# AMReX-Combustion/PeleAnalysis

Measured on AMD Instinct MI355X. Metric: Mcells/s for grad+curvature on 512^3-base 3-level AMR; % HBM roofline, higher is better.
Workload: dtype f64; 1 GPU; fused grad->curvature, 3-level AMR, base 512^3, ref_ratio 2, 128^3 boxes (64 per level) in the file, swept on the internal tiling pa_level_retile makes of them (4, 4, 4 boxes per level, largest 512x256x256), 1 comp(s), periodic x/y + wall z, 402653184 cells in the job; cells=402653184, cells_this_rank=402653184, ncomp=1, components_per_batch=1, fused=True, parallelism=single GPU

## Files before the change

### peleanalysis_amd/csrc/pa_core.hip

```cpp
#include "pa_internal.h"
#include "pa_dist.h"
#include <algorithm>
#include <atomic>
#include <cstring>
#include <numeric>

int pa_fail(pa_ctx* ctx, const std::string& msg) {
  if (ctx) ctx->err = msg;
  return 1;
}

int pa_ensure_scr(pa_ctx* ctx, size_t bytes, int slot) {
  void*& p = slot ? ctx->d_scr2 : ctx->d_scr;
  size_t& cap = slot ? ctx->scr2_cap : ctx->scr_cap;
  if (cap >= bytes) return 0;
  if (p) (void)hipFree(p);
  p = nullptr;
  cap = 0;
  PA_HIP(hipMalloc(&p, bytes));
  cap = bytes;
  return 0;
}

extern "C" int pa_version(void) { return 100; }

static int host_owner(const pa_level* L, int i, int j, int k);
const WgTab* pa_sweep_wgtab(const pa_level* L, int cls, int tw, int mty, int kseg, bool force, int part) {
  if (part) force = true;
  const long long key = ((long long)cls << 56) | ((long long)part << 54) | ((long long)(force ? 1 : 0) << 52) | ((long long)tw << 40) | ((long long)mty << 24) | (long long)kseg;
  auto it = L->wgtabs.find(key);
  if (it != L->wgtabs.end()) return (it->second->d || part) ? it->second.get() : nullptr;
  std::unique_ptr<WgTab> T(new WgTab());
  struct Chunk { int n, box, t0; };
  std::vector<std::pair<int, int>> bt;
  std::vector<std::vector<int>> sel;
  long long real = 0;
  int tmax = 0;
  std::vector<unsigned char> sp;
  if (part) {
    sp.assign(L->boxes.size(), 0);
    for (int f : L->sfaces) sp[(size_t)(f / 6)] |= (unsigned char)(1u << (f % 6));
  }
  for (int b = 0; b < (int)L->boxes.size(); ++b) {
    const DBox& B = L->boxes[b];
    const int nx = B.hi[0] - B.lo[0] + 1, ny = B.hi[1] - B.lo[1] + 1, nz = B.hi[2] - B.lo[2] + 1;
    if (cls != 2 && (nx <= 32) != (cls == 1)) continue;
    const int tx = (nx + tw - 1) / tw, ty = (ny + mty - 1) / mty, tz = (nz + kseg - 1) / kseg;
    int t = tx * ty * tz;
    if (part) {
      std::vector<int> mine;
      for (int id = 0; id < t; ++id) {
        const int bx = id % tx, by = (id / tx) % ty, bz = id / (tx * ty);
        int lo[3] = {B.lo[0] + bx * tw, B.lo[1] + by * mty, B.lo[2] + bz * kseg}, hi[3];
        hi[0] = std::min(lo[0] + tw - 1, B.hi[0]); hi[1] = std::min(lo[1] + mty - 1, B.hi[1]); hi[2] = std::min(lo[2] + kseg - 1, B.hi[2]);
        bool early = true;
        for (int d = 0; d < 3 && early; ++d) {
          if (((sp[(size_t)b] >> (2 * d)) & 1) && lo[d] == B.lo[d]) early = false;
          if (((sp[(size_t)b] >> (2 * d + 1)) & 1) && hi[d] >= B.hi[d] - 1) early = false;
        }
        for (int d = 0; d < 3 && early; ++d)
          for (int side = 0; side < 2 && early; ++side) {
            int slo[3], shi[3];
            for (int q = 0; q < 3; ++q) { slo[q] = std::max(lo[q] - 2, B.lo[q] - 2); shi[q] = std::min(hi[q] + 2, B.hi[q] + 2); }
            if (side == 0) shi[d] = std::min(shi[d], B.lo[d] - 1); else slo[d] = std::max(slo[d], B.hi[d] + 1);
            if (slo[d] > shi[d]) continue;
            for (int k = slo[2]; k <= shi[2] && early; ++k)
              for (int j = slo[1]; j <= shi[1] && early; ++j)
                for (int i = slo[0]; i <= shi[0]; ++i)
                  if (host_owner(L, i, j, k) < 0) { early = false; break; }
          }
        if (early == (part == 1)) mine.push_back(id);
      }
      t = (int)mine.size();
      if (t == 0) continue;
      sel.push_back(std::move(mine));
    }
    bt.push_back({t, b});
    real += t;
    tmax = std::max(tmax, t);
  }
  const long long launched = (long long)tmax * 8 * (((long long)bt.size() + 7) / 8);
  if (!bt.empty()) {
    constexpr int chunk_env = 0;
    const int cap = chunk_env > 0 ? chunk_env : (int)std::max<long long>(8, std::min<long long>(64, real / 32));
    std::vector<Chunk> ch;
    for (size_t bi = 0; bi < bt.size(); ++bi) {
      const auto& p = bt[bi];
      const int parts = (p.first + cap - 1) / cap;
      for (int q = 0; q < parts; ++q) {
        const int a = (int)((long long)p.first * q / parts), e = (int)((long long)p.first * (q + 1) / parts);
        ch.push_back({e - a, part ? (int)bi : p.second, a});
      }
    }
    std::stable_sort(ch.begin(), ch.end(), [](const Chunk& a, const Chunk& b) { return a.n > b.n; });
    std::vector<Chunk> queue[8];
    long long load[8] = {0, 0, 0, 0, 0, 0, 0, 0};
    for (const Chunk& c : ch) {
      int q = 0;
      for (int x = 1; x < 8; ++x)
        if (load[x] < load[q]) q = x;
      queue[q].push_back(c);
      load[q] += c.n;
    }
    const long long qlen = *std::max_element(load, load + 8);
    if (force || launched * 100 > qlen * 8 * 103) {
      std::vector<int> tab((size_t)(qlen * 8 * 2), 0);
      for (int q = 0; q < 8; ++q) {
        long long s = 0;
        for (const Chunk& c : queue[q])
          for (int t = 0; t < c.n; ++t, ++s) {
            tab[(size_t)(2 * (8 * s + q))] = part ? bt[(size_t)c.box].second : c.box;
            tab[(size_t)(2 * (8 * s + q) + 1)] = part ? sel[(size_t)c.box][(size_t)(c.t0 + t)] : c.t0 + t;
          }
        for (; s < qlen; ++s) tab[(size_t)(2 * (8 * s + q))] = -1;
      }
      if (hipMalloc(&T->d, sizeof(int) * tab.size()) == hipSuccess && hipMemcpy(T->d, tab.data(), sizeof(int) * tab.size(), hipMemcpyHostToDevice) == hipSuccess) {
        T->n = (unsigned)(tab.size() / 2);
        T->h = std::move(tab);
      } else {
        if (T->d) (void)hipFree(T->d);
        T->d = nullptr;
        (void)hipGetLastError();
      }
    }
  }
  const WgTab* raw = T.get();
  L->wgtabs[key] = std::move(T);
  return (raw->d || part) ? raw : nullptr;
}

const unsigned char* pa_sweep_gneed(const pa_level* L, const WgTab* T, int tw, int mty, int kseg, long long fine_serial, const std::vector<int>* cpregs) {
  if (!T || !T->d || T->h.size() != 2 * (size_t)T->n) return nullptr;
  auto it = T->gneed.find(fine_serial);
  if (it != T->gneed.end()) return it->second;
  const int nb = (int)L->boxes.size();
  pa_level* Lm = const_cast<pa_level*>(L);
  if ((int)Lm->xneed.size() != nb) {
    std::vector<unsigned char> sp((size_t)nb, 0);
    for (int f : L->sfaces) sp[(size_t)(f / 6)] |= (unsigned char)(1u << (f % 6));
    Lm->xneed.assign((size_t)nb, 0);
    for (int b = 0; b < nb; ++b) {
      const DBox& B = L->boxes[b];
      for (int side = 0; side < 2; ++side) {
        bool need = (sp[(size_t)b] >> side) & 1;
        const int x = side ? B.hi[0] + 1 : B.lo[0] - 1;
        int last = -1;
        for (int k = B.lo[2]; k <= B.hi[2] && !need; k += L->g)
          for (int j = B.lo[1]; j <= B.hi[1] && !need; j += L->g) {
            const int o = host_owner(L, x, j, k);
            if (o < 0 || o == last) continue;
            last = o;
            const DBox& N = L->boxes[o];
            if ((sp[(size_t)o] >> (1 - side)) & 1) need = true;
            for (int d = 1; d < 3 && !need; ++d)
              for (int t = 0; t < 2; ++t) {
                const int c = t ? N.hi[d] : N.lo[d];
                if (((sp[(size_t)o] >> (2 * d + t)) & 1) && c >= B.lo[d] + 3 && c <= B.hi[d] - 3) need = true;
              }
          }
        if (need) Lm->xneed[(size_t)b] |= (unsigned char)(2u << side);
      }
    }
  }
  std::vector<std::vector<unsigned char>> full((size_t)nb);
  auto tiles = [&](const DBox& B, int& tx, int& ty, int& tz) {
    tx = (B.hi[0] - B.lo[0] + tw) / tw; ty = (B.hi[1] - B.lo[1] + mty) / mty; tz = (B.hi[2] - B.lo[2] + kseg) / kseg;
  };
  if (cpregs)
    for (size_t r = 0; r + 12 <= cpregs->size(); r += 12) {
      const int* R = cpregs->data() + r;
      const int sb = R[1], dir = R[9], t0 = dir == 0 ? 1 : 0, t1 = dir == 2 ? 1 : 2;
      if (sb < 0 || sb >= nb) continue;
      const DBox& B = L->boxes[sb];
      int lo[3] = {R[4], R[5], R[6]}, hi[3] = {R[4], R[5], R[6]};
      hi[t0] += R[7] - 1; hi[t1] += R[8] - 1;
      int tx, ty, tz;
      tiles(B, tx, ty, tz);
      auto& F = full[(size_t)sb];
      if (F.empty()) F.assign((size_t)tx * ty * tz, 0);
      const int a0 = std::max(0, (lo[0] - B.lo[0]) / tw), a1 = std::min(tx - 1, (hi[0] - B.lo[0]) / tw);
      const int b0 = std::max(0, (lo[1] - B.lo[1]) / mty), b1 = std::min(ty - 1, (hi[1] - B.lo[1]) / mty);
      const int c0 = std::max(0, (lo[2] - B.lo[2]) / kseg), c1 = std::min(tz - 1, (hi[2] - B.lo[2]) / kseg);
      for (int c = c0; c <= c1; ++c)
        for (int bb = b0; bb <= b1; ++bb)
          for (int a = a0; a <= a1; ++a) F[((size_t)c * ty + bb) * tx + a] = 1;
    }
  std::vector<unsigned char> need((size_t)T->n, 0);
  for (unsigned e = 0; e < T->n; ++e) {
    const int b = T->h[2 * (size_t)e], id = T->h[2 * (size_t)e + 1];
    if (b < 0 || b >= nb) continue;
    unsigned char v = Lm->xneed[(size_t)b];
    if (!full[(size_t)b].empty() && id >= 0 && (size_t)id < full[(size_t)b].size() && full[(size_t)b][(size_t)id]) v |= 1;
    need[(size_t)e] = v;
  }
  unsigned char* d = nullptr;
  if (hipMalloc(&d, need.size()) != hipSuccess || hipMemcpy(d, need.data(), need.size(), hipMemcpyHostToDevice) != hipSuccess) {
    if (d) (void)hipFree(d);
    (void)hipGetLastError();
    return nullptr;
  }
  T->gneed[fine_serial] = d;
  return d;
}

static pa_options g_opt;
static bool g_opt_read = false;
extern "C" void pa_options_reload(void) {
  pa_options o;
  auto geti = [](const char* n, int def) { const char* e = getenv(n); return e ? atoi(e) : def; };
  o.filter_exact = geti("PA_FILTER_EXACT", 0) != 0;
  o.allow_unverified_gaussian = geti("PA_ALLOW_UNVERIFIED_GAUSSIAN", 0) != 0;
  if (const char* e = getenv("PA_RETILE_MAX")) {
    int v[3] = {0, 0, 0};
    if (sscanf(e, "%d %d %d", &v[0], &v[1], &v[2]) == 3 && v[0] > 0 && v[1] > 0 && v[2] > 0)
      for (int d = 0; d < 3; ++d) o.retile_max[d] = v[d];
  }
  o.fused2 = geti("PA_FUSED2", 1) != 0;
  o.ncg = geti("PA_NCG", 1) != 0;
  o.dist_early = geti("PA_DIST_EARLY", 0) != 0;
  o.smooth_replicated = geti("PA_SMOOTH_REPLICATED", 0) != 0;
  o.smooth_mg = geti("PA_SMOOTH_MG", -1);
  o.smooth_march = geti("PA_SMOOTH_MARCH", 1) != 0;
  o.smooth_timing = geti("PA_SMOOTH_TIMING", 0) != 0;
  o.force_fallbacks = geti("PA_FORCE_FALLBACKS", 0) != 0;
  o.scratch_poison = geti("PA_SCRATCH_POISON", 0) != 0;
  g_opt = o;
  g_opt_read = true;
}
const pa_options& pa_opt() {
  if (!g_opt_read) pa_options_reload();
  return g_opt;
}

extern "C" pa_ctx* pa_ctx_create(int device, void* hip_stream) {
  int ndev = 0;
  if (hipGetDeviceCount(&ndev) != hipSuccess || ndev <= 0 || device >= ndev) return nullptr;
  if (hipSetDevice(device) != hipSuccess) return nullptr;
  pa_ctx* ctx = new pa_ctx();
  ctx->device = device;
  if (hip_stream) {
    ctx->stream = (hipStream_t)hip_stream;
  } else {
    if (hipStreamCreate(&ctx->stream) != hipSuccess) { delete ctx; return nullptr; }
    ctx->own_stream = true;
  }
  if (hipMalloc(&ctx->d_flags, 16 * sizeof(int)) != hipSuccess || hipMemset(ctx->d_flags, 0, 16 * sizeof(int)) != hipSuccess) {
    if (ctx->own_stream) (void)hipStreamDestroy(ctx->stream);
    delete ctx;
    return nullptr;
  }
  if (hipStreamCreateWithFlags(&ctx->stream2, hipStreamNonBlocking) != hipSuccess) { ctx->stream2 = nullptr; (void)hipGetLastError(); }
  return ctx;
}

extern "C" void pa_ctx_destroy(pa_ctx* ctx) {
  PaBind bind_(ctx);
  if (!ctx) return;
  pa_rccl_destroy(ctx);
  if (ctx->d_red) (void)hipFree(ctx->d_red);
  if (ctx->d_flags) (void)hipFree(ctx->d_flags);
  if (ctx->d_slow) (void)hipFree(ctx->d_slow);
  if (ctx->d_prog) (void)hipFree(ctx->d_prog);
  for (hipEvent_t e : ctx->fix_evs)
    if (e) (void)hipEventDestroy(e);
  if (ctx->d_scr) (void)hipFree(ctx->d_scr);
  if (ctx->d_scr2) (void)hipFree(ctx->d_scr2);
  if (ctx->h_pin) (void)hipHostFree(ctx->h_pin);
  if (ctx->d_mcz) (void)hipFree(ctx->d_mcz);
  if (ctx->d_flat_nosrc) (void)hipFree(ctx->d_flat_nosrc);
  for (auto& c : ctx->surf_cache) (void)hipFree(c.first);
  for (auto& e : ctx->evs) { (void)hipEventDestroy(e.a); (void)hipEventDestroy(e.b); }
  for (auto& e : ctx->sync_evs) (void)hipEventDestroy(e);
  if (ctx->stream2) (void)hipStreamDestroy(ctx->stream2);
  for (auto& st : ctx->lev_streams) (void)hipStreamDestroy(st);
  if (ctx->own_stream) (void)hipStreamDestroy(ctx->stream);
  delete ctx;
}

extern "C" int pa_profile_enable(pa_ctx* ctx, int on) {
  PaBind bind_(ctx);
  if (!ctx) return 1;
// ... 1103 lines not shown
```

### peleanalysis_amd/csrc/pa_internal.h

```cpp
#pragma once
#include <hip/hip_runtime.h>
#include <cstdint>
#include <array>
#include <map>
#include <memory>
#include <string>
#include <utility>
#include <vector>
#include "../../include/peleanalysis_amd.h"

struct DBox { int lo[3]; int hi[3]; };

struct pa_options {
  int filter_exact = 0;
  int allow_unverified_gaussian = 0;
  int retile_max[3] = {0, 0, 0};
  int fused2 = 1;
  int ncg = 1;
  int dist_early = 0;
  int smooth_replicated = 0;
  int smooth_mg = -1;
  int smooth_march = 1;
  int smooth_timing = 0;
  int scratch_poison = 0;
// ... 37 lines not shown

struct DMFView {
  double* data;
  const long long* off;
  int ncomp, ng;
  int xform;
  double xa, xb;
};

#define PA_MAXB 4
#define PA_MAXSLOTS 16
template <typename A, int CAP = PA_MAXB>
struct LevBatch {
  int n = 0;
  int ycum[CAP + 1] = {};
  A a[CAP];
  __device__ __forceinline__ int find(unsigned y, unsigned& local) const {
    int l = 0;
    while (l + 1 < n && y >= (unsigned)ycum[l + 1]) ++l;
    local = y - (unsigned)ycum[l];
    return l;
  }
};

struct pa_ctx {
  int device = 0;
  hipStream_t stream = nullptr;
  bool own_stream = false;
  std::string err;
  double* d_red = nullptr;
  size_t red_cap = 0;
  int* d_flags = nullptr;
  void* d_slow = nullptr;
  hipEvent_t fix_evs[2] = {nullptr, nullptr};
  double* d_prog = nullptr;
  void* d_scr = nullptr;
  size_t scr_cap = 0;
  void* d_scr2 = nullptr;
  size_t scr2_cap = 0;
  void* h_pin = nullptr;
  size_t h_pin_cap = 0;
  void* d_mcz = nullptr;
  size_t mcz_cap = 0;
  bool mcz_dirty = true;
  std::map<void*, size_t> surf_live;
  std::vector<std::pair<void*, size_t>> surf_cache;
  unsigned profile = 0;
  struct Ev { hipEvent_t a, b; int tag; };
  std::vector<Ev> evs;
  hipStream_t stream2 = nullptr;
  std::vector<hipStream_t> lev_streams;
  std::vector<hipEvent_t> sync_evs;
  std::string sweep_kernel;
  int smooth_iters = -1;
  double smooth_res = 0.0;
  int curv_path = -1;
  unsigned long long* d_flat_nosrc = nullptr;
  int32_t filter_info[8] = {0, 0, 0, 0, 0, 0, 0, 0};
  pa_comm comm = {nullptr, 0, 1, nullptr, nullptr};
  struct RcclState* rccl = nullptr;
};

struct ProfScope {
  pa_ctx* ctx;
  pa_ctx::Ev e;
  bool on;
  ProfScope(pa_ctx* c, int tag) : ctx(c), on(((c->profile >> tag) & 1u) != 0) {
    if (!on) return;
    e.tag = tag;
    if (hipEventCreate(&e.a) != hipSuccess || hipEventCreate(&e.b) != hipSuccess) { on = false; return; }
    (void)hipEventRecord(e.a, ctx->stream);
  }
  ~ProfScope() {
    if (!on) return;
    (void)hipEventRecord(e.b, ctx->stream);
    ctx->evs.push_back(e);
  }
};
enum { PA_TAG_GRADCURV = 1, PA_TAG_GRADCURV_FACES = 2, PA_TAG_FILL = 3, PA_TAG_BC = 4, PA_TAG_GRAD = 5, PA_TAG_PROGRESS = 6,
       PA_TAG_FILTER = 7, PA_TAG_MC = 8, PA_TAG_XCHG = 9 };

struct WgTab {
  int* d = nullptr;
  unsigned n = 0;
  std::vector<int> h;
  mutable std::map<long long, unsigned char*> gneed;
  ~WgTab() {
    if (d) (void)hipFree(d);
    for (auto& kv : gneed)
      if (kv.second) (void)hipFree(kv.second);
  }
};

struct pa_level {
  pa_ctx* ctx = nullptr;
  std::vector<DBox> boxes;
  int domlo[3], domhi[3], is_per[3];
  double prob_lo[3], prob_hi[3], dx[3], dxinv[3];
  int g = 1, mlo[3], mn[3];
  std::vector<int> owner;
  DBox* d_boxes = nullptr;
  int* d_owner = nullptr;
  std::vector<int> sfaces;
  int* d_sfaces = nullptr;
  int* d_sfindex = nullptr;
  long long* d_sfoff = nullptr;
  unsigned short* d_sfcode = nullptr;
  int maxn[3] = {0, 0, 0};
  long long ncells = 0;
  bool fusable = true;
  bool pure_faces = true;
  long long* d_cpoff = nullptr;
  double* d_cp = nullptr;
  int cp_sets = 0, cg_sets = 0;
  long long cp_total = 0;
  long long* d_cgoff = nullptr;
  double* d_cg = nullptr;
  long long cg_total = 0;
  double* d_ncg = nullptr;
  bool ncg_live = false;
  int ncg_minw = 0;
  std::vector<long long> cgoff;
  int* d_blist = nullptr;
  int nwide = 0, nnarrow = 0;
  int wmax[3] = {0, 0, 0}, nmax[3] = {0, 0, 0};
  int* d_sfboxes = nullptr;
  int nsfboxes = 0;
  void* d_sfwg = nullptr;
  int nsfwg = 0;
  void* d_pfwg = nullptr;
  int npfwg = 0;
  SfChunk* d_sfchunk = nullptr;
  int nsfchunk = 0;
  void* d_ring = nullptr;
  int nring = -1;
  std::vector<unsigned char> xneed;
  void* d_irr = nullptr;
  int nirr = -1;
  int nremote = 0;
  DLevelView view;
  int rank = 0, nranks = 1;
  long long serial = 0;
  std::vector<DBox> gboxes;
  std::vector<int> gowner;
  std::vector<int> gid;
  std::vector<int> glocal;
  bool source_only = false;
  mutable std::map<int, std::unique_ptr<struct XPlan>> fb_plans;
  mutable std::map<long long, std::unique_ptr<struct CpPlan>> cp_plans;
  mutable std::map<int, std::unique_ptr<struct FbLocal>> fb_local;
  mutable std::map<std::pair<long long, int>, std::unique_ptr<struct CsPlan>> cs_plans;
  mutable std::unique_ptr<struct RepPlan> rep_plan;
  mutable std::map<long long, std::unique_ptr<WgTab>> wgtabs;
  mutable std::map<long long, std::unique_ptr<struct RsPlan>> rs_plans;
  mutable std::map<std::pair<long long, int>, std::unique_ptr<struct FpPlan>> fp_plans;
  mutable std::map<std::array<long long, 5>, std::unique_ptr<struct FlPlan>> fl_plans;
  mutable std::map<std::array<int, 3>, struct pa_mf*> scratch;
  ~pa_level();
};

struct FpPlan {
  int n = 0;
  void* d_items = nullptr;
  ~FpPlan();
};

struct FlPlan {
  int nwide = 0, ngeneral = 0, nskipped = 0, nrect = 0;
  int nptile = 0, notile = 0, ngtile = 0;
  void* d_ptile = nullptr;
  void* d_rects = nullptr;
  void* d_otile = nullptr;
  int* d_glist = nullptr;
  ~FlPlan();
};

struct LevelSpec {
  std::vector<DBox> local;
  std::vector<int> gid;
  std::vector<DBox> gboxes;
  std::vector<int> gowner;
  int rank = 0, nranks = 1;
  bool source_only = false;
};
pa_level* pa_level_create_spec(pa_ctx* ctx, const LevelSpec& S, const int32_t domlo[3], const int32_t domhi[3], const int32_t is_per[3],
                               const double prob_lo[3], const double prob_hi[3]);
bool pa_face_is_special(const pa_level* L, const DBox& B, int d, int side);
struct pa_mf* pa_level_scratch(pa_ctx* ctx, const pa_level* L, int ncomp, int ng, int role = 0);
const WgTab* pa_sweep_wgtab(const pa_level* L, int cls, int tw, int mty, int kseg, bool force, int part = 0);
const unsigned char* pa_sweep_gneed(const pa_level* L, const WgTab* T, int tw, int mty, int kseg, long long fine_serial, const std::vector<int>* cpregs);
int pa_host_classify(const pa_level* L, int i, int j, int k);

struct pa_mf {
  const pa_level* lev = nullptr;
  int ncomp = 0, ng = 0;
  double* data = nullptr;
  bool owned = false;
  std::vector<long long> off;
  long long* d_off = nullptr;
  long long total = 0;
  DMFView view;
};

#define PA_HIP(call)                                                                      \
  do {                                                                                    \
    hipError_t e_ = (call);                                                               \
    if (e_ != hipSuccess) {                                                               \
      ctx->err = std::string(#call) + ": " + hipGetErrorString(e_);                       \
      return 1;                                                                           \
    }                                                                                     \
  } while (0)

int pa_fail(pa_ctx* ctx, const std::string& msg);

int pa_ensure_red(pa_ctx* ctx, size_t n);
int pa_ensure_scr(pa_ctx* ctx, size_t bytes, int slot = 0);
int pa_fill_boundary_impl(pa_ctx* ctx, pa_mf* M, int comp, int ncomp, int ng, int no_exchange);
int pa_fill_boundary_local_batch(pa_ctx* ctx, int n, pa_mf* const* Ms, int comp, int ncomp, int ng);
int pa_fill_boundary_local_batch_ngs(pa_ctx* ctx, int n, pa_mf* const* Ms, int comp, int ncomp, const int* ngs);
int pa_apply_bc_impl(pa_ctx* ctx, pa_mf* F, int comp, const pa_mf* C, int ccomp, const int32_t bc[3], int ratio, int only_dir,
                     int edges, const double* crse_xform);
int pa_apply_bc_dual(pa_ctx* ctx, pa_mf* F0, int comp0, pa_mf* F1, int comp1, const pa_mf* C, int ccomp, const int32_t bc[3], int ratio,
                     const double* xform);
int pa_grad_levels(pa_ctx* ctx, int nlev, pa_mf* const* phi, int comp, pa_mf* const* out, int ocomp);
int pa_gauss_curv_level(pa_ctx* ctx, const pa_mf* G, int gcomp, const pa_mf* normgrad, int ngcomp, const pa_mf* c, int ccomp, double thr, pa_mf* out,
                        int kcomp);
int pa_strain_level(pa_ctx* ctx, const pa_mf* u, int ucomp, pa_mf* out, int srcomp, int rostcomp);
int pa_velnormal_level(pa_ctx* ctx, const pa_mf* u, int ucomp, const pa_mf* n, int ncomp0, const pa_mf* c, int ccomp, double thr, pa_mf* out, int ocomp);
int pa_curvopts_level(pa_ctx* ctx, int which, const pa_mf* G, const pa_mf* u, int ucomp, pa_mf* out, int pc, int nc, int kgc, int src, int vnc, int rostc, double thr);
int pa_gradcurv_prep_levels(pa_ctx* ctx, int nlev, pa_mf* const* phi, int comp, const pa_mf* const* crse, int ccomp, const int32_t bc[3], double pmin, double pmax, int phase = 3,
                            int nslots = 1, const double* prog = nullptr);
int pa_poison_level_caches(pa_ctx* ctx, int nlev, pa_mf* const* state);
int pa_poison_mf(pa_ctx* ctx, pa_mf* m);
bool pa_gradcurv_gout_ok(int nlev, pa_mf* const* phi);
bool pa_gradcurv_parts_ok(int nlev, pa_mf* const* phi);
bool pa_gradcurv_kg_ok(int nlev, pa_mf* const* phi);
int pa_gradcurv_levels_cg(pa_ctx* ctx, int nlev, pa_mf* const* phi, int pcomp, double pmin, double pmax, pa_mf* const* out, int ocomp, double thr = -1.0, int slot = 0,
                          int nslots = 1, const double* prog = nullptr, const double* pmins = nullptr, const double* pmaxs = nullptr, pa_mf* const* gout = nullptr, int part = 0, int kg = 0);
int pa_gradcurv_faces_phase(pa_ctx* ctx, const pa_mf* c, int ccomp, const pa_mf* crse_n, int cncomp0, const int32_t bc[3], int ratio, double thr,
                            pa_mf* out, int ncomp0, int kcomp, int phase);
int pa_gradcurv_fix_levels(pa_ctx* ctx, int nlev, pa_mf* const* phi, int pcomp, const pa_mf* const* crse_n, int cncomp0, const int32_t bc[3], double pmin, double pmax,
                           pa_mf* const* out, int ncomp0, int kcomp, double thr = -1.0, int nslots = 1, const double* prog = nullptr, int cn_z = 8,
                           const pa_mf* const* crse_phi = nullptr, int cpcomp = 0);
bool pa_fused2_level_ok(const pa_level* L);
int pa_gauss_cells_levels(pa_ctx* ctx, int nlev, pa_mf* const* G, pa_mf* const* out, int pc, int kgc, double thr);
std::vector<double> pa_binmef_edges(double bmin, double bmax, int n);
long long pa_binmef_slice(const int* cr, long long n, long long cap, long long* tot);

struct PaBind {
  explicit PaBind(const pa_ctx* c) { if (c) (void)hipSetDevice(c->device); }
};

__host__ __device__ __forceinline__ long long pa_cstride(long long ncells, int ncomp) {
  long long cs = (ncells + 63) / 64 * 64;
  if (ncomp > 1) {
    if (ncells >= 32768) cs += (256 + 2048 - cs % 2048) % 2048;
    else if ((cs % 2048) == 0) cs += 64;
  }
  return cs;
}

__device__ __forceinline__ long long fab_index(const DBox& B, int ng, int ncomp, int c, int i, int j, int k) {
  const long long nx = B.hi[0] - B.lo[0] + 1 + 2 * ng, ny = B.hi[1] - B.lo[1] + 1 + 2 * ng,
                  nz = B.hi[2] - B.lo[2] + 1 + 2 * ng;
  return (long long)c * pa_cstride(nx * ny * nz, ncomp) + ((long long)(k - B.lo[2] + ng) * ny + (j - B.lo[1] + ng)) * nx + (i - B.lo[0] + ng);
}

__device__ __forceinline__ bool wrap_cell(const DLevelView& L, int p[3]) {
#pragma unroll
  for (int d = 0; d < 3; ++d) {
    const int len = L.domhi[d] - L.domlo[d] + 1;
    if (p[d] < L.domlo[d] || p[d] > L.domhi[d]) {
      if (!L.is_per[d]) return false;
      while (p[d] < L.domlo[d]) p[d] += len;
      while (p[d] > L.domhi[d]) p[d] -= len;
    }
  }
  return true;
}

__device__ __forceinline__ int owner_of(const DLevelView& L, const int p[3]) {
  int m[3];
#pragma unroll
  for (int d = 0; d < 3; ++d) {
    const int r = p[d] - L.mlo[d];
    if (r < 0) return -1;
    m[d] = L.gshift >= 0 ? (r >> L.gshift) : (r / L.g);
    if (m[d] >= L.mn[d]) return -1;
  }
  return L.owner[((long long)m[2] * L.mn[1] + m[1]) * L.mn[0] + m[0]];
}

__device__ __forceinline__ int classify(const DLevelView& L, int i, int j, int k, int& box, int p[3]) {
  p[0] = i; p[1] = j; p[2] = k;
  if (!wrap_cell(L, p)) return 2;
  box = owner_of(L, p);
  return (box != -1) ? 0 : 1;
}
__device__ __forceinline__ int classify(const DLevelView& L, int i, int j, int k) {
  int b, p[3];
  return classify(L, i, j, k, b, p);
}

__host__ __device__ __forceinline__ int coarsen_idx(int i, int r) { return r == 2 ? (i >> 1) : ((i < 0) ? -((-i + r - 1) / r) : i / r); }

template <typename F>
__device__ __forceinline__ double sg_sum(const double n[3], F f) {
  return +n[0] * n[1] * n[2] * f(1, 1, 1)
         + n[0] * (1.0 - n[1]) * n[2] * f(1, 0, 1)
         + n[0] * n[1] * (1.0 - n[2]) * f(1, 1, 0)
         + n[0] * (1.0 - n[1]) * (1.0 - n[2]) * f(1, 0, 0)
         + (1.0 - n[0]) * n[1] * n[2] * f(0, 1, 1)
         + (1.0 - n[0]) * (1.0 - n[1]) * n[2] * f(0, 0, 1)
         + (1.0 - n[0]) * n[1] * (1.0 - n[2]) * f(0, 1, 0)
         + (1.0 - n[0]) * (1.0 - n[1]) * (1.0 - n[2]) * f(0, 0, 0);
}

__device__ __forceinline__ void poly_interp_coeff(double xInt, const double* x, int N, double* c) {
  for (int j = 0; j < N; ++j) {
    double num = 1.0, den = 1.0;
    for (int i = 0; i < N; ++i) {
      if (i == j) continue;
      num *= xInt - x[i];
      den *= x[j] - x[i];
    }
    c[j] = num / den;
  }
}

__device__ __forceinline__ double cdiff(double dxinv, double m, double c, double p) {
  const double fl = -(dxinv * (c - m));
  const double fh = -(dxinv * (p - c));
  return -(0.5 * (fl + fh));
}

__device__ __forceinline__ double crse_raw(const DLevelView& LC, const DMFView& MC, int comp, int ic, int jc, int kc, bool& ok) {
  int p[3] = {ic, jc, kc};
  if (!wrap_cell(LC, p)) { ok = false; return 0.0; }
  const int b = owner_of(LC, p);
  if (b < 0) { ok = false; return 0.0; }
  return MC.data[MC.off[b] + fab_index(LC.boxes[b], MC.ng, MC.ncomp, comp, p[0], p[1], p[2])];
}
// ... 219 lines not shown
```

### peleanalysis_amd/csrc/pa_stencil.hip

```cpp
#include "pa_internal.h"
#include "pa_fabview.h"
#include "pa_grad_march.h"
#include <algorithm>
#include <cfloat>
#include <cstdlib>

template <typename BP>
static void grad_launch(hipStream_t st, const BP& bp, int nx, int ny, int nz, unsigned nboxes, int comp, int ocomp, const pa_level* L = nullptr) {
  constexpr int kseg_env = 16, mty_env = 0;
  const bool tables = L != nullptr;
  auto table = [&](int cls, int tw, int mty, int kseg, bool force) -> const WgTab* { return tables ? pa_sweep_wgtab(L, cls, tw, mty, kseg, force) : nullptr; };
  auto wide = [&](int wx, int wy, int wz, int cls, bool force) {
    GradMarchArgs A{comp, ocomp, std::max(1, std::min(kseg_env, wz)), (int)nboxes, 0};
    const int mty = mty_env ? mty_env : (wy >= 52 ? 13 : (wy >= 16 ? 8 : 4));
    auto go = [&](auto tyc) {
      constexpr int M = decltype(tyc)::value;
      A.tiles_max = ((wx + 63) / 64) * ((wy + M - 1) / M) * ((wz + A.kseg - 1) / A.kseg);
      const WgTab* wt = table(cls, 64, M, A.kseg, force);
      if (wt) A.wgtab = wt->d;
      const dim3 g(wt ? wt->n : (unsigned)A.tiles_max * 8u * ((nboxes + 7u) / 8u));
      hipLaunchKernelGGL((k_grad_march<BP, M>), g, dim3(64 * (M + 3)), 0, st, bp, A);
    };
    switch (mty) {
      case 13: go(std::integral_constant<int, 13>{}); break;
      case 8: go(std::integral_constant<int, 8>{}); break;
      case 5: go(std::integral_constant<int, 5>{}); break;
      default: go(std::integral_constant<int, 4>{}); break;
    }
  };
  auto narrow = [&](int wx, int wy, int wz, int cls, bool force) {
    constexpr int NRW = 8;
    GradMarchArgs A{comp, ocomp, std::max(1, std::min(kseg_env, wz)), (int)nboxes, 0};
    A.tiles_max = ((wx + 31) / 32) * ((wy + 2 * NRW - 1) / (2 * NRW)) * ((wz + A.kseg - 1) / A.kseg);
    const WgTab* wt = table(cls, 32, 2 * NRW, A.kseg, force);
    if (wt) A.wgtab = wt->d;
    const dim3 g(wt ? wt->n : (unsigned)A.tiles_max * 8u * ((nboxes + 7u) / 8u));
    hipLaunchKernelGGL((k_grad_marchn<BP, NRW>), g, dim3(64 * (NRW + 2)), 0, st, bp, A);
  };
  if (tables && L->nwide && L->nnarrow) {
    wide(L->wmax[0], L->wmax[1], L->wmax[2], 0, true);
    narrow(L->nmax[0], L->nmax[1], L->nmax[2], 1, true);
    return;
  }
  if (nx > 32) wide(nx, ny, nz, 2, false);
  else narrow(nx, ny, nz, 2, false);
}

extern "C" int pa_grad_level(pa_ctx* ctx, const pa_mf* phi, int comp, pa_mf* out, int ocomp) {
  PaBind bind_(ctx);
  if (!ctx || !phi || !out) return pa_fail(ctx, "pa_grad_level: null argument");
  if (phi->lev != out->lev) return pa_fail(ctx, "pa_grad_level: phi and out live on different levels");
  if (phi->ng < 1) return pa_fail(ctx, "pa_grad_level: phi needs >= 1 ghost layer");
  if (comp < 0 || comp >= phi->ncomp || ocomp < 0 || ocomp + 4 > out->ncomp) return pa_fail(ctx, "pa_grad_level: component range");
  LevelBP2 bp{phi->lev->view, phi->view, out->view};
  const pa_level* L = phi->lev;
  if (phi->lev->boxes.empty()) return 0;
  ProfScope prof(ctx, PA_TAG_GRAD);
  grad_launch(ctx->stream, bp, L->maxn[0], L->maxn[1], L->maxn[2], (unsigned)L->boxes.size(), comp, ocomp, L);
  PA_HIP(hipGetLastError());
  return 0;
}

int pa_grad_levels(pa_ctx* ctx, int nlev, pa_mf* const* phi, int comp, pa_mf* const* out, int ocomp) {
  if (nlev < 2 || pa_opt().force_fallbacks) return -1;
  for (int l = 0; l < nlev; ++l) {
    const pa_level* L = phi[l]->lev;
    if (L->boxes.empty()) continue;
    if (L->nnarrow > 0 || L->maxn[1] < 52) return -1;
    for (const DBox& B : L->boxes)
      if (B.hi[0] - B.lo[0] + 1 <= 32) return -1;
  }
  for (int l0 = 0; l0 < nlev; l0 += PA_MAXB) {
  GradBatch S;
  S.n = 0;
  S.wg0[0] = 0;
  for (int l = l0; l < nlev && l < l0 + PA_MAXB; ++l) {
    const pa_level* L = phi[l]->lev;
    if (L->boxes.empty()) continue;
    GradMarchArgs A{comp, ocomp, std::max(1, std::min(16, L->maxn[2])), (int)L->boxes.size(), 0};
    A.tiles_max = ((L->maxn[0] + 63) / 64) * ((L->maxn[1] + 12) / 13) * ((L->maxn[2] + A.kseg - 1) / A.kseg);
    const WgTab* wt = pa_sweep_wgtab(L, 2, 64, 13, A.kseg, false);
    if (wt) A.wgtab = wt->d;
    S.bp[S.n] = LevelBP2{L->view, phi[l]->view, out[l]->view};
    S.A[S.n] = A;
    S.wg0[S.n + 1] = S.wg0[S.n] + (wt ? wt->n : (unsigned)A.tiles_max * 8u * (((unsigned)L->boxes.size() + 7u) / 8u));
    ++S.n;
  }
  if (!S.n) continue;
  ProfScope prof(ctx, PA_TAG_GRAD);
  hipLaunchKernelGGL(k_grad_march_levels<13>, dim3(S.wg0[S.n]), dim3(64 * 16), 0, ctx->stream, S);
  PA_HIP(hipGetLastError());
  }
  return 0;
}

extern "C" int pa_grad_fab(pa_ctx* ctx, pa_box valid, const pa_fab* phi, int comp, const double dxinv[3], pa_fab* out, int ocomp) {
  PaBind bind_(ctx);
  if (!ctx || !phi || !out || !dxinv) return pa_fail(ctx, "pa_grad_fab: null argument");
  std::string why;
  if (!fab_covers(*phi, valid, 1, comp, 1, why) || !fab_covers(*out, valid, 0, ocomp, 4, why)) return pa_fail(ctx, "pa_grad_fab: " + why);
  FabBP2 bp{fab_view(*phi), fab_view(*out), to_dbox(valid), {dxinv[0], dxinv[1], dxinv[2]}};
  grad_launch(ctx->stream, bp, valid.hi[0] - valid.lo[0] + 1, valid.hi[1] - valid.lo[1] + 1, valid.hi[2] - valid.lo[2] + 1, 1, comp, ocomp);
  PA_HIP(hipGetLastError());
  return 0;
}

__global__ __launch_bounds__(256) void k_minmax(DLevelView L, DMFView M, int comp, double* part) {
  const int b = blockIdx.y;
  const DBox B = L.boxes[b];
  const int nx = B.hi[0] - B.lo[0] + 1, ny = B.hi[1] - B.lo[1] + 1, nz = B.hi[2] - B.lo[2] + 1;
  const long long n = (long long)nx * ny * nz;
  double lo = DBL_MAX, hi = -DBL_MAX;
  const double* f = M.data + M.off[b];
  for (long long t = blockIdx.x * (long long)blockDim.x + threadIdx.x; t < n; t += (long long)gridDim.x * blockDim.x) {
    const int i = (int)(t % nx), j = (int)((t / nx) % ny), k = (int)(t / ((long long)nx * ny));
    const double v = f[fab_index(B, M.ng, M.ncomp, comp, B.lo[0] + i, B.lo[1] + j, B.lo[2] + k)];
    lo = v < lo ? v : lo;
    hi = v > hi ? v : hi;
  }
  for (int o = 32; o > 0; o >>= 1) {
    const double l2 = __shfl_xor(lo, o), h2 = __shfl_xor(hi, o);
    lo = l2 < lo ? l2 : lo;
    hi = h2 > hi ? h2 : hi;
  }
  __shared__ double slo[4], shi[4];
  const int w = threadIdx.x >> 6;
  if ((threadIdx.x & 63) == 0) { slo[w] = lo; shi[w] = hi; }
  __syncthreads();
  if (threadIdx.x == 0) {
    for (int q = 1; q < 4; ++q) { lo = slo[q] < lo ? slo[q] : lo; hi = shi[q] > hi ? shi[q] : hi; }
    const long long slot = (long long)blockIdx.y * gridDim.x + blockIdx.x;
    part[2 * slot] = lo;
    part[2 * slot + 1] = hi;
  }
}

extern "C" int pa_minmax_level(pa_ctx* ctx, const pa_mf* s, int comp, double* mn, double* mx) {
  PaBind bind_(ctx);
  if (!ctx || !s || !mn || !mx) return pa_fail(ctx, "pa_minmax_level: null argument");
  if (comp < 0 || comp >= s->ncomp) return pa_fail(ctx, "pa_minmax_level: component range");
  const unsigned nb = (unsigned)s->lev->boxes.size();
  const unsigned gx = 32;
  if (nb == 0) { *mn = DBL_MAX; *mx = -DBL_MAX; return 0; }
  if (pa_ensure_red(ctx, 2 * (size_t)gx * nb)) return 1;
  hipLaunchKernelGGL(k_minmax, dim3(gx, nb), dim3(256), 0, ctx->stream, s->lev->view, s->view, comp, ctx->d_red);
  PA_HIP(hipGetLastError());
  std::vector<double> h(2 * (size_t)gx * nb);
  PA_HIP(hipMemcpyAsync(h.data(), ctx->d_red, h.size() * sizeof(double), hipMemcpyDeviceToHost, ctx->stream));
  PA_HIP(hipStreamSynchronize(ctx->stream));
  double lo = DBL_MAX, hi = -DBL_MAX;
  for (size_t q = 0; q < h.size(); q += 2) { lo = std::min(lo, h[q]); hi = std::max(hi, h[q + 1]); }
  *mn = lo;
  *mx = hi;
  return 0;
}

template <typename BP>
__global__ __launch_bounds__(256) void k_progress(BP bp, int comp, int ccomp, double pmin, double invdenom) {
  FabView S, C;
  DBox V;
  double dxinv[3];
  if (!bp.get(blockIdx.y, S, C, V, dxinv)) return;
  int i, j, k0, k1;
  if (!tile_cell(V, i, j, k0, k1)) return;
  for (int k = k0; k <= k1; ++k) C(i, j, k, ccomp) = (S(i, j, k, comp) - pmin) * invdenom;
}

extern "C" int pa_progress_level(pa_ctx* ctx, const pa_mf* s, int comp, double pmin, double pmax, pa_mf* c, int ccomp, int ng) {
  PaBind bind_(ctx);
  if (!ctx || !s || !c) return pa_fail(ctx, "pa_progress_level: null argument");
  if (s->lev != c->lev) return pa_fail(ctx, "pa_progress_level: different levels");
  if (ng > s->ng || ng > c->ng || comp >= s->ncomp || ccomp >= c->ncomp) return pa_fail(ctx, "pa_progress_level: ng/component range");
  const double invdenom = 1.0 / (pmax - pmin);
  if (s->lev->boxes.empty()) return 0;
  LevelBP2 bp{s->lev->view, s->view, c->view, ng};
  ProfScope prof(ctx, PA_TAG_PROGRESS);
  hipLaunchKernelGGL(k_progress<LevelBP2>, tile_grid(s->lev, ng), dim3(256), 0, ctx->stream, bp, comp, ccomp, pmin, invdenom);
  PA_HIP(hipGetLastError());
  return 0;
}

extern "C" int pa_progress_fab(pa_ctx* ctx, pa_box bx, const pa_fab* s, int comp, double pmin, double pmax, pa_fab* c, int ccomp) {
  PaBind bind_(ctx);
  if (!ctx || !s || !c) return pa_fail(ctx, "pa_progress_fab: null argument");
  std::string why;
  if (!fab_covers(*s, bx, 0, comp, 1, why) || !fab_covers(*c, bx, 0, ccomp, 1, why)) return pa_fail(ctx, "pa_progress_fab: " + why);
  const double invdenom = 1.0 / (pmax - pmin);
  FabBP2 bp{fab_view(*s), fab_view(*c), to_dbox(bx), {1, 1, 1}};
  hipLaunchKernelGGL(k_progress<FabBP2>, tile_grid(bx), dim3(256), 0, ctx->stream, bp, comp, ccomp, pmin, invdenom);
  PA_HIP(hipGetLastError());
  return 0;
}

template <typename BP>
__global__ __launch_bounds__(256) void k_normal(BP bp, int comp, int gcomp, int ngcomp, int ncomp0) {
  FabView C, G, NG, N;
  DBox V;
  double dxinv[3];
  if (!bp.get(blockIdx.y, C, G, NG, N, V, dxinv)) return;
  int i, j, k0, k1;
  if (!tile_cell(V, i, j, k0, k1)) return;
  double zm = C(i, j, k0 - 1, comp), zc = C(i, j, k0, comp);
  for (int k = k0; k <= k1; ++k) {
    const double zp = C(i, j, k + 1, comp);
    const double gx = cdiff(dxinv[0], C(i - 1, j, k, comp), zc, C(i + 1, j, k, comp));
    const double gy = cdiff(dxinv[1], C(i, j - 1, k, comp), zc, C(i, j + 1, k, comp));
    const double gz = cdiff(dxinv[2], zm, zc, zp);
    const double sn = sqrt(gx * gx + gy * gy + gz * gz);
    const double ng = -((1e-14 < sn) ? sn : 1e-14);
    if (G.p) { G(i, j, k, gcomp) = gx; G(i, j, k, gcomp + 1) = gy; G(i, j, k, gcomp + 2) = gz; }
    if (NG.p) NG(i, j, k, ngcomp) = ng;
    N(i, j, k, ncomp0) = gx / ng;
    N(i, j, k, ncomp0 + 1) = gy / ng;
    N(i, j, k, ncomp0 + 2) = gz / ng;
    zm = zc;
    zc = zp;
  }
}

extern "C" int pa_normal_level(pa_ctx* ctx, const pa_mf* c, int comp, pa_mf* G, int gcomp, pa_mf* normgrad, int ngcomp,
                               pa_mf* n, int ncomp0) {
  PaBind bind_(ctx);
  if (!ctx || !c || !n) return pa_fail(ctx, "pa_normal_level: null argument");
  if (c->ng < 1) return pa_fail(ctx, "pa_normal_level: c needs >= 1 ghost layer");
  if (c->lev != n->lev || (G && G->lev != c->lev) || (normgrad && normgrad->lev != c->lev)) return pa_fail(ctx, "pa_normal_level: different levels");
  if (comp >= c->ncomp || ncomp0 + 3 > n->ncomp || (G && gcomp + 3 > G->ncomp) || (normgrad && ngcomp >= normgrad->ncomp))
    return pa_fail(ctx, "pa_normal_level: component range");
  DMFView none{nullptr, nullptr, 0, 0};
  if (c->lev->boxes.empty()) return 0;
  LevelBP4 bp{c->lev->view, c->view, G ? G->view : none, normgrad ? normgrad->view : none, n->view};
  hipLaunchKernelGGL(k_normal<LevelBP4>, tile_grid(c->lev), dim3(256), 0, ctx->stream, bp, comp, gcomp, ngcomp, ncomp0);
  PA_HIP(hipGetLastError());
// ... 84 lines not shown
```

Before: 73230 Mcells/s.

## Choose grad march z-segment length with a wave-count cost model

Factors the workgroup-table dealing into a shared header and adds a cached per-level queue-length estimate. The gradient launches then pick the z-segment length (kseg) from candidates up to the full box depth, using a cost model that trades wave count against per-segment fill overhead. Longer segments cut redundant halo plane loads and per-segment startup in the marching kernel. The cost is fewer workgroups and a possible load-balance tail.

After: 73240 Mcells/s, median of 3. Within noise of the previous version (+0.0%).

```diff
diff --git a/peleanalysis_amd/csrc/pa_core.hip b/peleanalysis_amd/csrc/pa_core.hip
--- a/peleanalysis_amd/csrc/pa_core.hip
+++ b/peleanalysis_amd/csrc/pa_core.hip
@@ -1,5 +1,6 @@
 #include "pa_internal.h"
 #include "pa_dist.h"
+#include "pa_wgtab.h"
 #include <algorithm>
 #include <atomic>
 #include <cstring>
@@ -31,10 +32,8 @@
   auto it = L->wgtabs.find(key);
   if (it != L->wgtabs.end()) return (it->second->d || part) ? it->second.get() : nullptr;
   std::unique_ptr<WgTab> T(new WgTab());
-  struct Chunk { int n, box, t0; };
-  std::vector<std::pair<int, int>> bt;
-  std::vector<std::vector<int>> sel;
-  long long real = 0;
+  std::vector<WgTabBox> bt;
+  std::vector<std::vector<int>> sel(part ? L->boxes.size() : 0);
   int tmax = 0;
   std::vector<unsigned char> sp;
   if (part) {
@@ -73,47 +72,18 @@
       }
       t = (int)mine.size();
       if (t == 0) continue;
-      sel.push_back(std::move(mine));
-    }
-    bt.push_back({t, b});
-    real += t;
+      sel[(size_t)b] = std::move(mine);
+    }
+    bt.push_back({b, {nx, ny, nz}, nullptr});
     tmax = std::max(tmax, t);
   }
+  if (part)
+    for (WgTabBox& B : bt) B.sel = &sel[(size_t)B.box];
   const long long launched = (long long)tmax * 8 * (((long long)bt.size() + 7) / 8);
   if (!bt.empty()) {
-    constexpr int chunk_env = 0;
-    const int cap = chunk_env > 0 ? chunk_env : (int)std::max<long long>(8, std::min<long long>(64, real / 32));
-    std::vector<Chunk> ch;
-    for (size_t bi = 0; bi < bt.size(); ++bi) {
-      const auto& p = bt[bi];
-      const int parts = (p.first + cap - 1) / cap;
-      for (int q = 0; q < parts; ++q) {
-        const int a = (int)((long long)p.first * q / parts), e = (int)((long long)p.first * (q + 1) / parts);
-        ch.push_back({e - a, part ? (int)bi : p.second, a});
-      }
-    }
-    std::stable_sort(ch.begin(), ch.end(), [](const Chunk& a, const Chunk& b) { return a.n > b.n; });
-    std::vector<Chunk> queue[8];
-    long long load[8] = {0, 0, 0, 0, 0, 0, 0, 0};
-    for (const Chunk& c : ch) {
-      int q = 0;
-      for (int x = 1; x < 8; ++x)
-        if (load[x] < load[q]) q = x;
-      queue[q].push_back(c);
-      load[q] += c.n;
-    }
-    const long long qlen = *std::max_element(load, load + 8);
+    const long long qlen = pa_wgtab_qlen(bt, tw, mty, kseg);
     if (force || launched * 100 > qlen * 8 * 103) {
-      std::vector<int> tab((size_t)(qlen * 8 * 2), 0);
-      for (int q = 0; q < 8; ++q) {
-        long long s = 0;
-        for (const Chunk& c : queue[q])
-          for (int t = 0; t < c.n; ++t, ++s) {
-            tab[(size_t)(2 * (8 * s + q))] = part ? bt[(size_t)c.box].second : c.box;
-            tab[(size_t)(2 * (8 * s + q) + 1)] = part ? sel[(size_t)c.box][(size_t)(c.t0 + t)] : c.t0 + t;
-          }
-        for (; s < qlen; ++s) tab[(size_t)(2 * (8 * s + q))] = -1;
-      }
+      std::vector<int> tab = pa_wgtab_build(bt, tw, mty, kseg);
       if (hipMalloc(&T->d, sizeof(int) * tab.size()) == hipSuccess && hipMemcpy(T->d, tab.data(), sizeof(int) * tab.size(), hipMemcpyHostToDevice) == hipSuccess) {
         T->n = (unsigned)(tab.size() / 2);
         T->h = std::move(tab);
@@ -127,6 +97,20 @@
   const WgTab* raw = T.get();
   L->wgtabs[key] = std::move(T);
   return (raw->d || part) ? raw : nullptr;
+}
+
+long long pa_sweep_qlen(const pa_level* L, int cls, int tw, int mty, int kseg) {
+  const long long key = ((long long)cls << 56) | ((long long)tw << 40) | ((long long)mty << 24) | (long long)kseg;
+  auto it = L->wgqlens.find(key);
+  if (it != L->wgqlens.end()) return it->second;
+  std::vector<WgTabBox> bt;
+  for (int b = 0; b < (int)L->boxes.size(); ++b) {
+    const DBox& B = L->boxes[b];
+    const int nx = B.hi[0] - B.lo[0] + 1;
+    if (cls != 2 && (nx <= 32) != (cls == 1)) continue;
+    bt.push_back({b, {nx, B.hi[1] - B.lo[1] + 1, B.hi[2] - B.lo[2] + 1}, nullptr});
+  }
+  return L->wgqlens[key] = pa_wgtab_qlen(bt, tw, mty, kseg);
 }
 
 const unsigned char* pa_sweep_gneed(const pa_level* L, const WgTab* T, int tw, int mty, int kseg, long long fine_serial, const std::vector<int>* cpregs) {
diff --git a/peleanalysis_amd/csrc/pa_internal.h b/peleanalysis_amd/csrc/pa_internal.h
--- a/peleanalysis_amd/csrc/pa_internal.h
+++ b/peleanalysis_amd/csrc/pa_internal.h
@@ -213,6 +213,7 @@
   mutable std::map<std::pair<long long, int>, std::unique_ptr<struct CsPlan>> cs_plans;
   mutable std::unique_ptr<struct RepPlan> rep_plan;
   mutable std::map<long long, std::unique_ptr<WgTab>> wgtabs;
+  mutable std::map<long long, long long> wgqlens;
   mutable std::map<long long, std::unique_ptr<struct RsPlan>> rs_plans;
   mutable std::map<std::pair<long long, int>, std::unique_ptr<struct FpPlan>> fp_plans;
   mutable std::map<std::array<long long, 5>, std::unique_ptr<struct FlPlan>> fl_plans;
@@ -249,6 +250,7 @@
 bool pa_face_is_special(const pa_level* L, const DBox& B, int d, int side);
 struct pa_mf* pa_level_scratch(pa_ctx* ctx, const pa_level* L, int ncomp, int ng, int role = 0);
 const WgTab* pa_sweep_wgtab(const pa_level* L, int cls, int tw, int mty, int kseg, bool force, int part = 0);
+long long pa_sweep_qlen(const pa_level* L, int cls, int tw, int mty, int kseg);
 const unsigned char* pa_sweep_gneed(const pa_level* L, const WgTab* T, int tw, int mty, int kseg, long long fine_serial, const std::vector<int>* cpregs);
 int pa_host_classify(const pa_level* L, int i, int j, int k);
 
diff --git a/peleanalysis_amd/csrc/pa_stencil.hip b/peleanalysis_amd/csrc/pa_stencil.hip
--- a/peleanalysis_amd/csrc/pa_stencil.hip
+++ b/peleanalysis_amd/csrc/pa_stencil.hip
@@ -1,9 +1,24 @@
 #include "pa_internal.h"
 #include "pa_fabview.h"
 #include "pa_grad_march.h"
+#include "pa_wgtab.h"
 #include <algorithm>
 #include <cfloat>
 #include <cstdlib>
+
+constexpr int PA_GRAD_KSEG = 16;
+static int grad_kseg(const std::vector<const pa_level*>& Ls, int cls, int mty) {
+  int nzmax = 0;
+  for (const pa_level* L : Ls) nzmax = std::max(nzmax, cls == 0 ? L->wmax[2] : L->maxn[2]);
+  auto places = [&](int k) {
+    long long n = 0;
+    for (const pa_level* L : Ls) n += pa_sweep_qlen(L, cls, 64, mty, k);
+    return n;
+  };
+  const int k0 = std::max(1, std::min(PA_GRAD_KSEG, nzmax));
+  if (places(k0) * 8 < 2048) return k0;
+  return pa_wgtab_kseg({PA_GRAD_KSEG, 32, 64, 128, nzmax}, nzmax, places);
+}
 
 template <typename BP>
 static void grad_launch(hipStream_t st, const BP& bp, int nx, int ny, int nz, unsigned nboxes, int comp, int ocomp, const pa_level* L = nullptr) {
@@ -11,8 +26,8 @@
   const bool tables = L != nullptr;
   auto table = [&](int cls, int tw, int mty, int kseg, bool force) -> const WgTab* { return tables ? pa_sweep_wgtab(L, cls, tw, mty, kseg, force) : nullptr; };
   auto wide = [&](int wx, int wy, int wz, int cls, bool force) {
-    GradMarchArgs A{comp, ocomp, std::max(1, std::min(kseg_env, wz)), (int)nboxes, 0};
     const int mty = mty_env ? mty_env : (wy >= 52 ? 13 : (wy >= 16 ? 8 : 4));
+    GradMarchArgs A{comp, ocomp, tables ? grad_kseg({L}, cls, mty) : std::max(1, std::min(kseg_env, wz)), (int)nboxes, 0};
     auto go = [&](auto tyc) {
       constexpr int M = decltype(tyc)::value;
       A.tiles_max = ((wx + 63) / 64) * ((wy + M - 1) / M) * ((wz + A.kseg - 1) / A.kseg);
@@ -71,13 +86,18 @@
       if (B.hi[0] - B.lo[0] + 1 <= 32) return -1;
   }
   for (int l0 = 0; l0 < nlev; l0 += PA_MAXB) {
+  std::vector<const pa_level*> Ls;
+  for (int l = l0; l < nlev && l < l0 + PA_MAXB; ++l)
+    if (!phi[l]->lev->boxes.empty()) Ls.push_back(phi[l]->lev);
+  if (Ls.empty()) continue;
+  const int kseg = grad_kseg(Ls, 2, 13);
   GradBatch S;
   S.n = 0;
   S.wg0[0] = 0;
   for (int l = l0; l < nlev && l < l0 + PA_MAXB; ++l) {
     const pa_level* L = phi[l]->lev;
     if (L->boxes.empty()) continue;
-    GradMarchArgs A{comp, ocomp, std::max(1, std::min(16, L->maxn[2])), (int)L->boxes.size(), 0};
+    GradMarchArgs A{comp, ocomp, std::min(kseg, L->maxn[2]), (int)L->boxes.size(), 0};
     A.tiles_max = ((L->maxn[0] + 63) / 64) * ((L->maxn[1] + 12) / 13) * ((L->maxn[2] + A.kseg - 1) / A.kseg);
     const WgTab* wt = pa_sweep_wgtab(L, 2, 64, 13, A.kseg, false);
     if (wt) A.wgtab = wt->d;
diff --git a/peleanalysis_amd/csrc/pa_wgtab.h b/peleanalysis_amd/csrc/pa_wgtab.h
--- /dev/null
+++ b/peleanalysis_amd/csrc/pa_wgtab.h
@@ -0,0 +1,79 @@
+#pragma once
+#include <algorithm>
+#include <vector>
+
+constexpr int PA_WG_QUEUES = 8;
+constexpr int PA_WG_RESIDENT = 32;
+
+struct WgTabBox {
+  int box;
+  int n[3];
+  const std::vector<int>* sel;
+};
+
+inline void pa_wgtab_tiles(const WgTabBox& B, int tw, int mty, int kseg, int& tx, int& ty, int& tz) {
+  tx = (B.n[0] + tw - 1) / tw; ty = (B.n[1] + mty - 1) / mty; tz = (B.n[2] + kseg - 1) / kseg;
+}
+
+inline long long pa_wgtab_box_count(const WgTabBox& B, int tw, int mty, int kseg) {
+  int tx, ty, tz;
+  pa_wgtab_tiles(B, tw, mty, kseg, tx, ty, tz);
+  return B.sel ? (long long)B.sel->size() : (long long)tx * ty * tz;
+}
+
+struct WgChunk { int n, bi, t0; };
+inline long long pa_wgtab_deal(const std::vector<WgTabBox>& boxes, int tw, int mty, int kseg, std::vector<WgChunk> (*queue)[PA_WG_QUEUES]) {
+  long long real = 0;
+  for (const WgTabBox& B : boxes) real += pa_wgtab_box_count(B, tw, mty, kseg);
+  const int cap = (int)std::max<long long>(8, std::min<long long>(2 * PA_WG_RESIDENT, real / 32));
+  std::vector<WgChunk> ch;
+  for (size_t bi = 0; bi < boxes.size(); ++bi) {
+    const long long t = pa_wgtab_box_count(boxes[bi], tw, mty, kseg);
+    const int parts = (int)((t + cap - 1) / cap);
+    for (int q = 0; q < parts; ++q) {
+      const int a = (int)(t * q / parts), e = (int)(t * (q + 1) / parts);
+      ch.push_back({e - a, (int)bi, a});
+    }
+  }
+  std::stable_sort(ch.begin(), ch.end(), [](const WgChunk& a, const WgChunk& b) { return a.n > b.n; });
+  long long load[PA_WG_QUEUES] = {0, 0, 0, 0, 0, 0, 0, 0};
+  for (const WgChunk& c : ch) {
+    int q = 0;
+    for (int x = 1; x < PA_WG_QUEUES; ++x)
+      if (load[x] < load[q]) q = x;
+    if (queue) (*queue)[q].push_back(c);
+    load[q] += c.n;
+  }
+  return *std::max_element(load, load + PA_WG_QUEUES);
+}
+inline long long pa_wgtab_qlen(const std::vector<WgTabBox>& boxes, int tw, int mty, int kseg) { return pa_wgtab_deal(boxes, tw, mty, kseg, nullptr); }
+
+inline std::vector<int> pa_wgtab_build(const std::vector<WgTabBox>& boxes, int tw, int mty, int kseg) {
+  std::vector<WgChunk> queue[PA_WG_QUEUES];
+  const long long qlen = pa_wgtab_deal(boxes, tw, mty, kseg, &queue);
+  std::vector<int> tab((size_t)(qlen * PA_WG_QUEUES * 2), 0);
+  for (int q = 0; q < PA_WG_QUEUES; ++q) {
+    long long s = 0;
+    for (const WgChunk& c : queue[q])
+      for (int t = 0; t < c.n; ++t, ++s) {
+        const WgTabBox& B = boxes[(size_t)c.bi];
+        tab[(size_t)(2 * (PA_WG_QUEUES * s + q))] = B.box;
+        tab[(size_t)(2 * (PA_WG_QUEUES * s + q) + 1)] = B.sel ? (*B.sel)[(size_t)(c.t0 + t)] : c.t0 + t;
+      }
+    for (; s < qlen; ++s) tab[(size_t)(2 * (PA_WG_QUEUES * s + q))] = -1;
+  }
+  return tab;
+}
+
+constexpr int PA_WG_FILL10 = 12, PA_WG_TAIL10 = 18;
+template <typename Places>
+inline int pa_wgtab_kseg(const std::vector<int>& cand, int nzmax, Places places) {
+  long long best = -1;
+  int best_k = 0;
+  for (int c : cand) {
+    const int k = std::max(1, std::min(c, nzmax));
+    const long long cost = ((places(k) + PA_WG_RESIDENT - 1) / PA_WG_RESIDENT) * (10 * k + PA_WG_FILL10) + (long long)PA_WG_TAIL10 * k;
+    if (best < 0 || cost < best) { best = cost; best_k = k; }
+  }
+  return best_k;
+}
```
